# ethereum/pos-evolution

Measured on AMD Instinct MI355X. Metric: attestations aggregated/sec + get_head() p50 latency at 1M validators, higher is better.
Workload: dtype int32

## Files before the change

pos_evolution_amd/csrc/att_bodies.inc:

```
#include <algorithm>
#include "att_rules.h"
#include "kernels.h"
#include "wave64.h"

namespace posevo {

namespace {

constexpr uint32_t VAL_EQUIVOCATING_BIT = 0x04u;
constexpr uint32_t ERR_INVALID_ARG = 1, ERR_CAPACITY = 10, ERR_NO_COMMITTEES = 11;

struct Row9 { uint4 q[9]; };
__device__ __forceinline__ void load_row(Row9& r, const uint4* __restrict__ rows, uint32_t i)
{
    const uint4* p = rows + (size_t)9 * i;
#pragma unroll
    for (int k = 0; k < 9; ++k) r.q[k] = p[k];
}
__device__ __forceinline__ unsigned long long u64_of(uint32_t lo, uint32_t hi) { return ((unsigned long long)hi << 32) | lo; }
__device__ __forceinline__ unsigned long long row_slot(const Row9& r) { return u64_of(r.q[0].x, r.q[0].y); }
__device__ __forceinline__ unsigned long long row_index(const Row9& r) { return u64_of(r.q[0].z, r.q[0].w); }
__device__ __forceinline__ unsigned long long row_source_epoch(const Row9& r) { return u64_of(r.q[3].x, r.q[3].y); }
__device__ __forceinline__ unsigned long long row_target_epoch(const Row9& r) { return u64_of(r.q[5].z, r.q[5].w); }

// ... 204 lines not shown
                if (stalled) break;
                const unsigned long long mi = __ballot(valid && have_incl);
                const int first = mi ? __builtin_ctzll(mi) : 64;
                const bool take = valid && (int)lane <= first;
                base.a += wave_sum(take ? x0 >> 1 : 0ull);
                base.w += wave_sum(take ? x1 >> 1 : 0ull);
                base.b += wave_sum(take ? x2 >> 1 : 0ull);
                if (mi) break;
                hi -= 64;
                if (hi < 0) break;
            }
            if (stalled && lane == 0) atomicMax(&a.sync->err, ERR_STALL);
            if (lane == 0) {
                granule_store(&rec[bid].incl[0], ((base.a + tot_a24) << 1) | 1ull);
                granule_store(&rec[bid].incl[1], ((base.w + tot.w) << 1) | 1ull);
                granule_store(&rec[bid].incl[2], ((base.b + tot.b) << 1) | 1ull);
            }
        }
        if (lane == 0) { s_base[0] = base.a; s_base[1] = base.w; s_base[2] = base.b; }
    }
    __syncthreads();

    uint32_t g = 0;
    if (is_rep) {
        const unsigned long long ex_a = wgb.a + inc.a - v.a;
        g = (uint32_t)(s_base[0] & 0xFFFFFFull) + (uint32_t)(ex_a & 0xFFFFull);
        const uint32_t list_start = (uint32_t)((s_base[0] >> 24) + (ex_a >> 16));
        const uint32_t out_word = (uint32_t)(s_base[1] + wgb.w + inc.w - v.w);
        const uint32_t out_byte = (uint32_t)(s_base[2] + wgb.b + inc.b - v.b);
        AttGroup G;
        G.rep = i;
        G.n_atts = natts;
        G.list_start = list_start;
        G.cursor = 0;
        G.n_bits = nbits;
        G.out_word = out_word;
        G.out_byte = out_byte;
        G.table = st == ST_NO_TABLE ? NONE32 : table;
        G.pos = pos;
        G.size = size;
        G.member_base = mbase;
        G.sig_valid = FLAG_SIG_VALID;
        G.status_agg = (uint32_t)st;
        G.index_over = index_over;
        G.pad[0] = G.pad[1] = 0;
        a.grp[g] = G;
        UnionGroup u;
        u.list_start = list_start;
        u.n_atts = natts;
        u.n_bits = nbits;
        u.out_word = out_word;
        a.ug[g] = u;
        a.gid_of_row[i] = g;
        if (ok) atomicAdd(&a.crow_cnt[table][pos], 1u);
    }
    {
        const int32_t st_pk = att_committee_state_status(st, index_over != 0);
        const uint32_t e = (is_rep && st_pk != ST_OK && a.want_pk) ? (st_pk == ST_NO_TABLE ? ERR_NO_COMMITTEES : ERR_INVALID_ARG) : 0u;
        const uint32_t w_err = wave_max(e);
        const uint32_t w_size = wave_max(ok ? size : 0u);
        const uint32_t w_mis = wave_max((is_rep && bytes != 4 * words) ? ~g : 0u);
        const uint32_t w_r0 = (uint32_t)__builtin_popcountll(__ballot(ok && table == 0));
        const uint32_t w_r1 = (uint32_t)__builtin_popcountll(__ballot(ok && table == 1));
        const unsigned long long w_mem = wave_sum(ok ? (unsigned long long)size : 0ull);
        if (lane == 0) {
            PlanSync* S = a.sync;
            if (w_err) atomicMax(&S->err, w_err);
            if (w_size) atomicMax(&S->max_size, w_size);
            if (w_mis) atomicMax(&S->mis_key, w_mis);
            if (w_r0) atomicAdd(&S->rows_t[0], w_r0);
            if (w_r1) atomicAdd(&S->rows_t[1], w_r1);
            if (w_mem) atomicAdd(&S->total_members, w_mem);
        }
    }

    asm volatile("s_waitcnt vmcnt(0)" ::: "memory");
    __syncthreads();
    if (tid == 0) s_ticket = __hip_atomic_fetch_add(&a.sync->ticket, 1u, __ATOMIC_RELAXED, __HIP_MEMORY_SCOPE_AGENT);
    __syncthreads();
    if (s_ticket != nb - 1) return;

    PlanSync* S = a.sync;
    const uint32_t rows_t0 = word_load(&S->rows_t[0]), rows_t1 = word_load(&S->rows_t[1]);
    if (tid == 0) {
        const unsigned long long la = granule_load(&rec[nb - 1].incl[0]) >> 1, lw = granule_load(&rec[nb - 1].incl[1]) >> 1,
                                 lb = granule_load(&rec[nb - 1].incl[2]) >> 1;
        const uint32_t ng = (uint32_t)(la & 0xFFFFFFull);
        const uint32_t max_size = word_load(&S->max_size), mis_key = word_load(&S->mis_key);
        const unsigned long long total_members = granule_load(&S->total_members);
        uint32_t err = max(a.plan->error, word_load(&S->err));
        if (!err && (lb > a.out_arena_cap || lw > 0xFFFFFFFFull)) err = ERR_CAPACITY;
        uint32_t k = a.min_k, L = 0;
        {
            const unsigned long long k0 = max((unsigned long long)a.min_k, (total_members + a.target_slots - 1) / a.target_slots);
            uint32_t tasks = (uint32_t)((max_size + k0 - 1) / k0);
            if (tasks > (uint32_t)G1_WG) tasks = G1_WG;
            while ((1u << L) < tasks) ++L;
            while (L > 0 && ((unsigned long long)ng << L) > a.slot_cap) --L;
            k = max(a.min_k, (max_size + (1u << L) - 1) >> L);
            if (k == 0) k = 1;
        }
        AttPlan p;
        p.n_groups = err ? 0u : ng;
        p.n_slots = p.n_groups << L;
        p.k = k;
        p.log2_block = L;
        p.out_words = (uint32_t)lw;
        p.out_bytes = (uint32_t)min(lb, 0xFFFFFFFFull);
        p.error = err;
        p.packed_same = (mis_key != 0 && (~mis_key) + 1 < ng) ? 0u : 1u;
        p.n_rows_table[0] = rows_t0;
        p.n_rows_table[1] = rows_t1;
        p.n_rows_in = n;
        p.last_error = err;
        p.total_members = total_members;
        *a.plan = p;
        *a.plan_host = p;
    }
    for (int t = 0; t < 2; ++t) {
        if (!a.tables.t[t].valid || (t ? rows_t1 : rows_t0) == 0) continue;
        const uint32_t nc = a.tables.t[t].n_committees;
        const uint32_t per = (nc + 1 + PLAN_WG - 1) / PLAN_WG;
        const uint32_t b0 = min(tid * per, nc + 1), b1 = min(b0 + per, nc + 1);
        uint32_t sum = 0;
        for (uint32_t c = b0; c < b1; ++c) sum += c < nc ? word_load(&a.crow_cnt[t][c]) : 0u;
        const uint32_t incl = wave_incl_scan(sum);
        __syncthreads();
        if (lane == 63) s_scan[wave] = incl;
        __syncthreads();
        uint32_t run = incl - sum;
        for (uint32_t w = 0; w < wave; ++w) run += s_scan[w];
        for (uint32_t c = b0; c < b1; ++c) {
            const uint32_t cnt = c < nc ? word_load(&a.crow_cnt[t][c]) : 0u;
            a.crow_start[t][c] = run;
            a.crow_cursor[t][c] = run;
            if (c < nc && cnt) __hip_atomic_store(&a.crow_cnt[t][c], 0u, __ATOMIC_RELAXED, __HIP_MEMORY_SCOPE_AGENT);
            run += cnt;
        }
    }
    __syncthreads();
    for (uint32_t j = tid; j < nb; j += PLAN_WG)
#pragma unroll
        for (int q = 0; q < 3; ++q) { granule_store(&rec[j].agg[q], 0ull); granule_store(&rec[j].incl[q], 0ull); }
    if (tid == 0) {
        unsigned long long* z = reinterpret_cast<unsigned long long*>(S);
#pragma unroll
        for (int q = 0; q < (int)(sizeof(PlanSync) / 8); ++q) granule_store(z + q, 0ull);
    }
}
inline unsigned att_plan_blocks(const AttPlanArgs& a) { return std::max(1u, (a.n + PLAN_WG - 1) / PLAN_WG); }
}

namespace {
__device__ __forceinline__ void att_members_body(const uint32_t i , const MembersArgs& a)
{
    const uint4* __restrict__ rows = static_cast<const uint4*>(a.rows);
    uint32_t* __restrict__ tab = a.tab;
    uint32_t* __restrict__ cnt_tab = a.cnt_tab;
    const uint32_t* __restrict__ slot_of = a.slot_of;
    const uint32_t* __restrict__ rep_of = a.rep_of;
    const uint32_t* __restrict__ gid_of_row = a.gid_of_row;
    AttGroup* __restrict__ grp = a.grp;
    AttPlan* __restrict__ plan = a.plan;
    uint32_t* __restrict__ ubytes = a.ubytes;
    uint32_t* __restrict__ member_row = a.member_row;
    uint32_t* __restrict__ host_group_of = a.host_group_of;
    uint4* __restrict__ host_out_rows = static_cast<uint4*>(a.host_out_rows);
    uint32_t n = a.n;
    if (a.n_dev) n = min(n, *a.n_dev);
    if (i == 0 && n == 0) plan->error = 0;
    if (i >= n) return;
    const uint32_t slot = slot_of[i];
    if (plan->n_groups) {
        const uint32_t rep = rep_of[i];
        const uint32_t g = gid_of_row[rep];
        const uint4 q8 = rows[(size_t)9 * i + 8];
        if (host_group_of) host_group_of[i] = g;
        AttGroup& G = grp[g];
        const uint32_t p = G.list_start + atomicAdd(&G.cursor, 1u);
        ubytes[p] = q8.x;
        member_row[p] = i;
        if (!(q8.z & FLAG_SIG_VALID)) atomicAnd(&G.sig_valid, 0u);
        if (rep == i) {
            const uint32_t k = plan->k, L = plan->log2_block;
            const bool ok = G.status_agg == (uint32_t)ST_OK;
            G1Group d;
            d.member_start = G.member_base;
            d.n_members = ok ? G.size : 0u;
            d.bits_word = G.out_word;
            d.slot_base = g << L;
            d.n_tasks = ok ? (G.size + k - 1) / k : 0u;
            d.k = k | (G.table == 1 ? 0x80000000u : 0u);
            d.log2_block = L;
            d.out_base = g;
            a.g1[g] = d;
            if (ok) a.crow_list[G.table][atomicAdd(&a.crow_cursor[G.table][G.pos], 1u)] = g;
            if (host_out_rows) {
                uint4* o = host_out_rows + (size_t)9 * g;
#pragma unroll
                for (int k8 = 0; k8 < 8; ++k8) o[k8] = rows[(size_t)9 * i + k8];
                o[8] = make_uint4(G.out_byte, q8.y, q8.z, 0u);
            }
        }
    }
    tab[slot] = ATT_EMPTY;
    cnt_tab[slot] = 0;
    if (i == 0) plan->error = 0;
}
}

namespace {
__device__ __forceinline__ uint32_t find_block_dev(const BlockTableDev& bt, const uint4& r0, const uint4& r1)
{
    uint32_t h = r0.x & bt.root_mask;
    for (;;) {
        const uint32_t idx = bt.root_tab[h];
        if (idx == NONE32) return NONE32;
        const uint4* q = reinterpret_cast<const uint4*>(bt.roots + 32ull * idx);
        if (same4(q[0], r0) && same4(q[1], r1)) return idx;
        h = (h + 1) & bt.root_mask;
    }
}
struct Root2 { uint4 lo, hi; };
struct BlockStoreDev {
    const BlockTableDev& bt;
    __device__ __forceinline__ uint32_t find(const Root2& r) const { return find_block_dev(bt, r.lo, r.hi); }
    __device__ __forceinline__ uint32_t handle(uint32_t idx) const { return bt.pos_of_idx[idx]; }
    __device__ __forceinline__ unsigned long long slot_of(uint32_t idx) const { return bt.slot_pos[bt.pos_of_idx[idx]]; }
    __device__ __forceinline__ uint32_t ancestor(uint32_t idx, unsigned long long slot) const
    {
        uint32_t p = bt.pos_of_idx[idx];
        while (bt.slot_pos[p] > slot && bt.parent_pos[p] != NONE32) p = bt.parent_pos[p];
        return p;
    }
};
}

namespace {
__device__ __forceinline__ void att_validate_fc_body(const uint32_t g , const ValidateFcArgs& a)
{
    const uint4* __restrict__ rows = static_cast<const uint4*>(a.rows);
    const AttGroup* __restrict__ grp = a.grp;
    const AttPlan* __restrict__ plan = a.plan;
    const uint32_t cap = a.cap;
    const BlockTableDev& bt = a.bt;
    const FcCtx& fc = a.fc;
    const uint32_t* __restrict__ union_info = a.union_info;
    AttRow* __restrict__ out_rows = a.out_rows;
    int32_t* __restrict__ status_dev = a.status_dev;
    int32_t* __restrict__ status_host = a.status_host;
    uint32_t* __restrict__ count_host = a.count_host;
    uint32_t* __restrict__ err_host = a.err_host;
    const uint32_t ng = plan->n_groups;
    if (ng > cap) {
        if (g < ng) status_dev[g] = -1;
        if (g == 0) *err_host = ERR_CAPACITY;
        return;
    }
    if (g >= ng) return;
    const AttGroup G = grp[g];
    Row9 r;
    load_row(r, rows, G.rep);
    const unsigned long long slot = row_slot(r), tep = row_target_epoch(r), spe = fc.slots_per_epoch;
    const FcVerdict v = att_fork_choice_status(BlockStoreDev{bt}, (r.q[8].z & FLAG_FROM_BLOCK) != 0, slot, tep, Root2{r.q[6], r.q[7]},
                                               Root2{r.q[1], r.q[2]}, fc.cur_slot, fc.cur_epoch, fc.prev_epoch, spe);
    int32_t st = v.status;
    if (st == ST_OK) st = (int32_t)G.status_agg;
    const uint32_t cnt = union_info[2 * g], overlap = union_info[2 * g + 1];
    if (st == ST_OK) st = att_indexed_status(G.sig_valid != 0, overlap != 0, cnt);
    out_rows[g] = att_row_fork_choice(G.member_base, G.size, G.out_word, v.block, tep, slot, g, g);
    status_dev[g] = st;
    status_host[g] = st;
    if (count_host) count_host[g] = st == ST_OK ? cnt : 0u;
}
}

namespace {
__device__ __forceinline__ void lmd_vm_tables_body(const unsigned long long v , const LmdVmArgs& a)
{
    const AttRow* __restrict__ rows = a.rows;
    const TablesDev& tables = a.tables;
    const uint32_t* __restrict__ cs0 = a.crow_start[0];
    const uint32_t* __restrict__ cs1 = a.crow_start[1];
    const uint32_t* __restrict__ cl0 = a.crow_list[0];
    const uint32_t* __restrict__ cl1 = a.crow_list[1];
    const AttPlan* __restrict__ plan = a.plan;
    const uint32_t* __restrict__ bit_arena = a.bit_arena;
    const uint8_t* __restrict__ flags = a.flags;
    unsigned long long* __restrict__ vote_key = reinterpret_cast<unsigned long long*>(a.vote_key);
    uint32_t* __restrict__ vote_block = a.vote_block;
    uint32_t* __restrict__ vote_slot = a.vote_slot;
    const uint32_t* __restrict__ gates = a.gates;
    if (v >= a.n_val) return;
    uint32_t best_e = 0, best_order = NONE32, new_block = NONE32, new_slot = 0;
    bool loaded = false;
    for (int t = 0; t < 2; ++t) {
        if (!tables.t[t].valid || plan->n_rows_table[t] == 0) continue;
        const uint32_t c = tables.t[t].inv_comm[v];
        if (c == NONE32) continue;
        const uint32_t* crow_start = t ? cs1 : cs0;
        const uint32_t* crow_list = t ? cl1 : cl0;
        const uint32_t kb = crow_start[c], ke = crow_start[c + 1];
        if (kb == ke) continue;
        if (!loaded) {
            if (flags[v] & VAL_EQUIVOCATING_BIT) return;
            best_e = (uint32_t)(vote_key[v] >> 32);
            loaded = true;
        }
        const uint32_t i = tables.t[t].inv_pos[v];
        for (uint32_t k = kb; k < ke; ++k) {
            const AttRow r = rows[crow_list[k]];
            if (i >= r.n_bits) continue;
            if (gates[r.gate] != 0) continue;
            if (!((bit_arena[r.bits_word + (i >> 5)] >> (i & 31)) & 1u)) continue;
            if (r.epoch_p1 > best_e || (r.epoch_p1 == best_e && new_block != NONE32 && r.order < best_order)) {
                best_e = r.epoch_p1;
                best_order = r.order;
                new_block = r.block_idx;
                new_slot = r.slot;
            }
        }
    }
    if (new_block != NONE32) {
        vote_key[v] = ((unsigned long long)best_e << 32) | 0xFFFFFFFFull;
        vote_block[v] = new_block;
        if (vote_slot) vote_slot[v] = new_slot;
    }
}
}

}
```

pos_evolution_amd/csrc/engine_resident.cpp:

```cpp
#include "engine_internal.h"


using namespace posevo;

namespace posevo {

namespace {

struct RrLayout {
    AttPlan* plan;
    uint32_t *slot_of, *rep_of, *gid_of_row, *ubytes, *member_row;
    PlanSync* sync;
    PlanRec* rec;
    AttGroup* grp;
    UnionGroup* ug;
    G1Group* g1;
    AttRow *rows_fc, *rows_st;
    int32_t *status_fc, *status_st;
    uint32_t* cmpl;
    uint32_t *crow_start[2], *crow_cursor[2], *crow_cnt[2], *crow_list[2];
    size_t bytes;
};

RrLayout rr_layout(uint8_t* base, uint32_t cap_n, uint32_t cap_c)
{
    RrLayout L;
    size_t off = 0;
    auto take = [&](size_t bytes) {
        uint8_t* p = base ? base + off : nullptr;
        off = (off + bytes + 255) & ~size_t(255);
        return p;
    };
    L.plan = reinterpret_cast<AttPlan*>(take(sizeof(AttPlan)));
    L.slot_of = reinterpret_cast<uint32_t*>(take(4ull * cap_n));
    L.rep_of = reinterpret_cast<uint32_t*>(take(4ull * cap_n));
    L.gid_of_row = reinterpret_cast<uint32_t*>(take(4ull * cap_n));
    L.sync = reinterpret_cast<PlanSync*>(take(sizeof(PlanSync)));
    L.rec = reinterpret_cast<PlanRec*>(take(sizeof(PlanRec) * ((size_t)cap_n / PLAN_WG + 1)));
    L.ubytes = reinterpret_cast<uint32_t*>(take(4ull * cap_n));
    L.member_row = reinterpret_cast<uint32_t*>(take(4ull * cap_n));
    L.grp = reinterpret_cast<AttGroup*>(take(sizeof(AttGroup) * (size_t)cap_n));
    L.ug = reinterpret_cast<UnionGroup*>(take(sizeof(UnionGroup) * (size_t)cap_n));
    L.g1 = reinterpret_cast<G1Group*>(take(sizeof(G1Group) * (size_t)cap_n));
    L.rows_fc = reinterpret_cast<AttRow*>(take(sizeof(AttRow) * (size_t)cap_n));
    L.rows_st = reinterpret_cast<AttRow*>(take(sizeof(AttRow) * (size_t)cap_n));
    L.status_fc = reinterpret_cast<int32_t*>(take(4ull * cap_n));
    L.status_st = reinterpret_cast<int32_t*>(take(4ull * cap_n));
    L.cmpl = reinterpret_cast<uint32_t*>(take(4ull * cap_n));
    for (int t = 0; t < 2; ++t) {
        L.crow_start[t] = reinterpret_cast<uint32_t*>(take(4ull * (cap_c + 1)));
        L.crow_cursor[t] = reinterpret_cast<uint32_t*>(take(4ull * (cap_c + 1)));
        L.crow_cnt[t] = reinterpret_cast<uint32_t*>(take(4ull * (cap_c + 1)));
        L.crow_list[t] = reinterpret_cast<uint32_t*>(take(4ull * cap_n));
    }
    L.bytes = off;
    return L;
}

struct RrSet {
    DevBuf &tab, &rr, &bits, &info;
    uint32_t &rows_cap, &comm_cap, &tab_size;
};
RrSet rr_set(pe_engine::PipeArena& a, int set)
{
    if (set == 0) return RrSet{a.d_rr_tab, a.d_rr, a.d_res_bits, a.d_res_info, a.rr_rows_cap, a.rr_comm_cap, a.rr_tab_size};
    return RrSet{a.x_rr_tab, a.x_rr, a.x_res_bits, a.x_res_info, a.x_rows_cap, a.x_comm_cap, a.x_tab_size};
}
RrLayout rr_of(pe_engine::PipeArena& a, int set = 0)
{
    const RrSet s = rr_set(a, set);
    return rr_layout(s.rr.as<uint8_t>(), s.rows_cap, s.comm_cap);
}

int rr_ensure(pe_engine* h, pe_engine::PipeArena& arena, int set, uint32_t n, uint32_t n_comm)
{
    {
        const RrSet rs = rr_set(arena, set);
        if (n <= rs.rows_cap && n_comm <= rs.comm_cap && rs.rr.p && rs.tab.p) return PE_OK;
    }
    PE_TRY(flush_pending(h));
    HIP_TRY(h, hipDeviceSynchronize());
    uint32_t cap_n = 1024, cap_c = 64;
    for (int i = 0; i < h->n_arenas; ++i) {
        const RrSet o = rr_set(h->arena[i], set);
        cap_n = std::max(cap_n, o.rows_cap);
        cap_c = std::max(cap_c, o.comm_cap);
    }
    while (cap_n < n) cap_n *= 2;
    while (cap_c < n_comm) cap_c *= 2;
    uint32_t tab = 2048;
    while (tab < 2 * cap_n) tab <<= 1;
    const RrLayout L = rr_layout(nullptr, cap_n, cap_c);
    for (int i = 0; i < h->n_arenas; ++i) {
        pe_engine::PipeArena& other = h->arena[i];
        if (set != 0 && &other != &arena) continue;
        const RrSet a = rr_set(other, set);
        if (cap_n <= a.rows_cap && cap_c <= a.comm_cap && a.rr.p && a.tab.p) continue;
        a.rr.release();
        a.tab.release();
        HIP_TRY(h, a.rr.ensure(L.bytes));
        HIP_TRY(h, a.tab.ensure(8ull * tab));
        HIP_TRY(h, hipMemsetAsync(a.tab.p, 0xFF, 4ull * tab, h->stream));
        HIP_TRY(h, hipMemsetAsync(a.tab.as<uint8_t>() + 4ull * tab, 0, 4ull * tab, h->stream));
        HIP_TRY(h, hipMemsetAsync(a.rr.p, 0, L.bytes, h->stream));
        a.rows_cap = cap_n;
        a.comm_cap = cap_c;
        a.tab_size = tab;
    }
    HIP_TRY(h, hipStreamSynchronize(h->stream));
    return PE_OK;
}

int candidate_tables(pe_engine* h, TablesDev* out, CommitteeTable* tabs[2])
{
    memset(out, 0, sizeof(*out));
    out->slots_per_epoch = h->cfg.slots_per_epoch;
    const uint64_t cur = epoch_at_slot(h, current_slot(h));
    const uint64_t prev = cur > 0 ? cur - 1 : cur;
    const uint64_t epochs[2] = {cur, prev};
    for (int k = 0; k < 2; ++k) {
        tabs[k] = nullptr;
        out->t[k].epoch = epochs[k];
        if (k == 1 && prev == cur) continue;
        CommitteeTable* t = find_table(h, epochs[k]);
        if (!t) continue;
        if (!t->is_partition || t->n_val_at_load != h->n_val || !t->d_inv_comm.p)
            return fail(h, PE_ERR_INVALID_ARG,
                        "rows in device memory: the committee tables of the current / previous epoch must partition the "
                        "registry they were loaded for (use host rows otherwise)");
        tabs[k] = t;
        out->t[k].members = t->d_members.as<uint32_t>();
        out->t[k].offsets = t->d_offsets.as<uint32_t>();
        out->t[k].inv_comm = t->d_inv_comm.as<uint32_t>();
        out->t[k].inv_pos = t->d_inv_pos.as<uint32_t>();
        out->t[k].n_committees = t->n_committees;
        out->t[k].valid = 1;
// ... 82 lines not shown
    OutBlock ob(h);
    const size_t off_plan = ob.alloc(sizeof(AttPlan));
    const size_t off_rows = ob.alloc(sizeof(pe_attestation) * (size_t)n);
    const size_t off_gof = ob.alloc(4ull * n);
    const size_t off_obits = ob.alloc(words_cap * 4);
    const size_t off_oinfo = ob.alloc(8ull * n);
    const size_t off_opk = out_aggpk96 ? ob.alloc(96ull * n) : 0;
    G1Complement cm;
    bool by_cmpl = false;
    if (out_aggpk96 && !dev_partials && set == 0 && h->tune.committee_sums && !h->dist_ready())
        for (int t = 0; t < 2; ++t) {
            if (tabs[t]) PE_TRY(committee_sums_build_wanted(h, tabs[t]));
            if (tabs[t] && tabs[t]->sums_valid && tabs[t]->d_sums.p && tabs[t]->ev_sums) {
                cm.sums[t] = tabs[t]->d_sums.as<uint32_t>();
                cm.ev[t] = tabs[t]->ev_sums;
                by_cmpl = true;
            }
        }
    const size_t off_ocm = by_cmpl ? ob.alloc(4ull * n) : 0;
    PE_TRY(ob.ensure());
    if (by_cmpl) {
        cm.cmpl = L.cmpl;
        cm.info = RS.info.as<uint32_t>();
    }
    if (want_pk) {
        PE_TRY(ensure_quiesced_arenas(h, &pe_engine::PipeArena::d_partials, std::max<size_t>(PE_G1_PARTIAL_BYTES, (size_t)PE_G1_PARTIAL_BYTES * n)));
        PE_TRY(ensure_quiesced_arenas(h, &pe_engine::PipeArena::d_lane_partials, (size_t)G1_LANE_PARTIAL_BYTES * slot_cap));
        PE_TRY(ensure_quiesced(h, h->d_partials, std::max<size_t>(PE_G1_PARTIAL_BYTES, (size_t)PE_G1_PARTIAL_BYTES * n)));
        PE_TRY(ensure_quiesced(h, h->d_lane_partials, (size_t)G1_LANE_PARTIAL_BYTES * slot_cap));
    }
    lap.mark("ragg.1_reserve");
    *out_n_groups = 0;
    AttPlan* plan_host = ob.host<AttPlan>(off_plan);
    memset(plan_host, 0, sizeof(AttPlan));
    plan_host->error = 0xFFFFFFFFu;
    const MemKind arena_kind = arena_len ? mem_kind(bits_arena) : MemKind::Pageable;
    hipStream_t ms = h->stream;
    const bool pair_ok = h->held.active && h->held.arena != h->cur && set == 0 && !n_dev && hold_eligible(h);
    if (h->held.active && !pair_ok) PE_TRY(held_issue(h));
    if (set == 0) {
        if (!h->deferred.empty()) PE_TRY(run_deferred(h));
        if (A.side_used) HIP_TRY(h, hipStreamWaitEvent(ms, h->ev_join, 0));
        if (sig_batch_holds(h, h->cur)) PE_TRY(sig_batch_flush(h));
        if (A.leg_used) HIP_TRY(h, hipStreamWaitEvent(ms, A.ev_leg, 0));
        PE_TRY(aux_join(h, ms));
    }
    h->res_valid = false;
    h->rr.valid = false;
    const size_t deferred_before = h->deferred.size();
    struct Unwind {
        pe_engine* h; size_t keep; bool armed = true;
        ~Unwind() { if (armed) { h->rr.valid = false; if (h->deferred.size() > keep) h->deferred.resize(keep); } }
    } unwind{h, deferred_before};
    bool ingest_copies = false;
    if (arena_kind == MemKind::Pageable) {
        memcpy(st.host<uint8_t>(off_arena), bits_arena, arena_len);
        memset(st.host<uint8_t>(off_arena) + arena_len, 0, pad_at + 32 - arena_len);
        HIP_TRY(h, st.upload());
    } else if (arena_len) {
        if (arena_kind == MemKind::Device && (reinterpret_cast<uintptr_t>(bits_arena) & 15) == 0 && n > 0) ingest_copies = true;
        else HIP_TRY(h, hipMemcpyAsync(st.dev<uint8_t>(off_arena), bits_arena, arena_len,
                                       arena_kind == MemKind::Device ? hipMemcpyDeviceToDevice : hipMemcpyHostToDevice, ms));
    }
    lap.mark("ragg.2_bits");
    uint32_t* cnt_tab = RS.tab.as<uint32_t>() + RS.tab_size;
    const IngestArgs ia{d_rows, n, RS.tab.as<uint32_t>(), cnt_tab, RS.tab_size - 1, L.slot_of, arena_len, L.plan,
                        st.dev<uint8_t>(off_arena) + pad_at, n_dev, ingest_copies ? bits_arena : nullptr,
                        ingest_copies ? st.dev<uint8_t>(off_arena) : nullptr};
    AttPlanArgs pa;
    pa.rows = d_rows;
    pa.n = n;
    pa.n_dev = n_dev;
    pa.tab = RS.tab.as<uint32_t>();
    pa.cnt_tab = cnt_tab;
    pa.slot_of = L.slot_of;
    pa.rep_of = L.rep_of;
    pa.gid_of_row = L.gid_of_row;
    pa.grp = L.grp;
    pa.ug = L.ug;
    for (int t = 0; t < 2; ++t) {
        pa.crow_start[t] = L.crow_start[t];
        pa.crow_cursor[t] = L.crow_cursor[t];
        pa.crow_cnt[t] = L.crow_cnt[t];
    }
    pa.sync = L.sync;
    pa.rec = L.rec;
    pa.plan = L.plan;
    pa.plan_host = plan_host;
    pa.out_arena_cap = out_arena_cap;
    pa.target_slots = target;
    pa.slot_cap = slot_cap;
    pa.min_k = G1_MIN_K;
    pa.want_pk = want_pk ? 1u : 0u;
    pa.tables = tables;
    const MembersArgs ma{d_rows, n, RS.tab.as<uint32_t>(), cnt_tab, L.slot_of, L.rep_of, L.gid_of_row, L.grp, L.plan, L.ubytes,
                         L.member_row, group_of ? ob.host<uint32_t>(off_gof) : nullptr, ob.host<uint8_t>(off_rows), n_dev,
                         L.g1, {L.crow_cursor[0], L.crow_cursor[1]}, {L.crow_list[0], L.crow_list[1]}};
    const UnionArgs ua{L.ug, n, L.ubytes, st.dev<uint8_t>(off_arena), RS.bits.as<uint32_t>(), RS.info.as<uint32_t>(),
                       ob.host<uint32_t>(off_obits), ob.host<uint32_t>(off_oinfo), L.plan,
                       by_cmpl ? L.cmpl : nullptr, by_cmpl ? ob.host<uint32_t>(off_ocm) : nullptr, L.grp,
                       {cm.sums[0] ? 1u : 0u, cm.sums[1] ? 1u : 0u}};
    PE_TRY(launch_rows_paired(h, ia, pa, ma, ua));
    HIP_TRY(h, hipGetLastError());
    lap.mark("ragg.3_group_union");
    if (want_pk) {
        const bool on_side = h->pipelining && h->side_stream && h->stream == h->own_stream;
        h->last_agg_on_side = on_side;
        pe_engine::PipeArena* arena = &A;
        const uint32_t* d_points = h->d_points.as<uint32_t>();
        const uint32_t* d_union = RS.bits.as<uint32_t>();
        uint8_t* out_pk = out_aggpk96 ? ob.host<uint8_t>(off_opk) : nullptr;
        G1Plan bound;
        bound.n_groups = n;
        bound.n_slots = slot_cap;
        bound.n_partials = n;
        const G1Group* d_groups = L.g1;
        const AttPlan* d_plan = L.plan;
        uint32_t* dev_jac = dev_partials ? dev_partials : set == 0 ? h->keep_pk : nullptr;
        auto launch_g1 = [h, arena, d_points, tables, d_union, d_groups, bound, out_pk, on_side, d_plan, dev_jac, cm, by_cmpl]() -> int {
            hipStream_t gs = on_side ? h->side_stream : h->stream;
            if (on_side) {
                HIP_TRY(h, hipEventRecord(h->ev_fork, h->stream));
                HIP_TRY(h, hipStreamWaitEvent(gs, h->ev_fork, 0));
            }
            if (on_side) {
                if (arena->side_used) HIP_TRY(h, hipStreamWaitEvent(gs, h->ev_join, 0));
            } else {
                g1_stream_guard(h, gs);
            }
            PE_TRY(launch_g1_planned(h, d_points, tables.t[0].members, d_union, d_groups, bound, out_pk, dev_jac, gs,
                                     on_side ? h->fin_stream : gs, on_side ? &arena->d_partials : nullptr,
                                     on_side ? &arena->d_lane_partials : nullptr, d_plan, tables.t[1].members, 0,
                                     by_cmpl ? &cm : nullptr));
            if (on_side) {
                HIP_TRY(h, hipEventRecord(h->ev_join, h->g1_tail()));
                h->side_busy = true;
                h->side_ever = true;
                arena->side_used = true;
            }
            return PE_OK;
        };
        if (on_side && h->streaming && !g1_chain_idle(h)) h->deferred.push_back(launch_g1);
        else PE_TRY(launch_g1());
        lap.mark("ragg.4_g1");
    }
    for (int t = 0; t < 2; ++t)
        if (tabs[t]) tabs[t]->stamp = ++h->table_stamp;
    unwind.armed = false;
    h->rr.valid = true;
    h->rr.arena = h->cur;
    h->rr.set = set;
    h->rr.n_in = n;
    h->rr.rows = d_rows;
    h->rr.tables = tables;
    ++h->rr.generation;
    h->rr.n_groups = NONE32;
    const size_t base = ob.base;
    const int ai = h->cur;
    const uint64_t gen = h->rr.generation;
    auto complete = [h, ai, base, off_plan, off_rows, off_gof, off_obits, off_oinfo, off_opk, off_ocm, by_cmpl, n, out_atts,
                     out_n_groups, group_of, out_bits_arena, out_aggpk96, out_count, gen]() -> int {
        const uint8_t* pin = h->arena[ai].h_pin.as<uint8_t>() + base;
        const AttPlan P = *reinterpret_cast<const AttPlan*>(pin + off_plan);
        if (P.error) return plan_error_to_status(h, P.error == 0xFFFFFFFFu ? 1u : P.error, "pe_aggregate (rows in device memory)");
        const uint32_t ng = P.n_groups;
        if (ng > n) return fail(h, PE_ERR_NO_DEVICE, "k_att_plan returned more groups than rows");
// ... 18 lines not shown
        h->last_cmpl_groups = 0;
        if (by_cmpl) {
            const uint32_t* ocm = reinterpret_cast<const uint32_t*>(pin + off_ocm);
            for (uint32_t g = 0; g < ng; ++g) h->last_cmpl_groups += ocm[g] != NONE32 ? 1u : 0u;
        }
        return PE_OK;
    };
    HostLap lap2(&h->trace);
    const int rc = finish_call(h, st, ob, complete);
    lap2.mark("ragg.5_wait_outputs");
    return rc;
}

int resident_plan_dev(pe_engine* h, const AttPlan** out)
{
    if (!h->rr.valid) return fail(h, PE_ERR_STATE, "no aggregate over rows in device memory on this handle");
    *out = rr_of(h->arena[h->rr.arena], h->rr.set).plan;
    return PE_OK;
}

int resident_parts(pe_engine* h, ResidentParts* out)
{
    if (!h->rr.valid) return fail(h, PE_ERR_STATE, "no aggregate over rows in device memory on this handle");
    pe_engine::PipeArena& RA = h->arena[h->rr.arena];
    const RrLayout L = rr_of(RA, h->rr.set);
    const RrSet RS = rr_set(RA, h->rr.set);
    out->rows = h->rr.rows;
    out->grp = L.grp;
    out->plan = L.plan;
    out->res_bits = RS.bits.as<uint32_t>();
    out->res_info = RS.info.as<uint32_t>();
    out->n_in = h->rr.n_in;
    return PE_OK;
}

int resident_lists(pe_engine* h, const UnionGroup** ug, const uint32_t** member_row)
{
    if (!h->rr.valid) return fail(h, PE_ERR_STATE, "no aggregate over rows in device memory on this handle");
    const RrLayout L = rr_of(h->arena[h->rr.arena], h->rr.set);
    *ug = L.ug;
    *member_row = L.member_row;
    return PE_OK;
}

int resident_precheck(pe_engine* h, const char* who)
{
    if (!h->rr.valid) return fail(h, PE_ERR_STATE, std::string(who) + ": PE_ROWS_RESIDENT without a pe_aggregate over rows in device memory on this handle");
    TablesDev now;
    CommitteeTable* tabs[2];
    PE_TRY(candidate_tables(h, &now, tabs));
    for (int t = 0; t < 2; ++t)
        if (now.t[t].epoch != h->rr.tables.t[t].epoch || now.t[t].valid != h->rr.tables.t[t].valid ||
            now.t[t].members != h->rr.tables.t[t].members)
            return fail(h, PE_ERR_STATE, std::string(who) + ": the store's clock or its committee tables changed since the resident pe_aggregate: aggregate again");
    return PE_OK;
}

int on_attestation_resident(pe_engine* h, uint32_t cap, int32_t* status, uint32_t* out_count)
{
    PE_TRY(resident_precheck(h, "pe_on_attestation_batch"));
    if (cap == 0) return PE_OK;
    if (h->held.active && (h->held.arena != h->cur || h->held.have_fc || h->held.have_head)) PE_TRY(held_issue(h));
    HostLap lap(&h->trace);
    PE_TRY(refresh_tree(h));
    pe_engine::PipeArena& RA = h->arena[h->rr.arena];
    const RrLayout L = rr_of(RA, h->rr.set);
    const RrSet RS = rr_set(RA, h->rr.set);
    Stage st(h);
    OutBlock ob(h);
    const size_t off_status = ob.alloc(4ull * cap);
    const size_t off_count = ob.alloc(4ull * cap);
    const size_t off_err = ob.alloc(16);
    PE_TRY(ob.ensure());
    *ob.host<uint32_t>(off_err) = 0;
    FcCtx fc;
    fc.cur_slot = current_slot(h);
    fc.cur_epoch = epoch_at_slot(h, fc.cur_slot);
    fc.prev_epoch = fc.cur_epoch > 0 ? fc.cur_epoch - 1 : 0;
    fc.slots_per_epoch = h->cfg.slots_per_epoch;
    const uint32_t n_launch = std::max<uint32_t>(h->rr.n_in, 1);
    memset(ob.host<int32_t>(off_status), 0, 4ull * cap);
    memset(ob.host<uint32_t>(off_count), 0, 4ull * cap);
    const ValidateFcArgs va{h->rr.rows, L.grp, L.plan, n_launch, cap, block_table_dev(h), fc, RS.info.as<uint32_t>(), L.rows_fc,
                            L.status_fc, ob.host<int32_t>(off_status), ob.host<uint32_t>(off_count), ob.host<uint32_t>(off_err)};
    const LmdVmArgs la{L.rows_fc, h->rr.tables, {L.crow_start[0], L.crow_start[1]}, {L.crow_list[0], L.crow_list[1]}, L.plan,
                       RS.bits.as<uint32_t>(), h->d_flags.as<uint8_t>(), h->n_val, h->d_vote_key.as<uint64_t>(),
                       h->d_vote_block.as<uint32_t>(), h->cfg.vote_expiry_slots ? h->d_vote_slot.as<uint32_t>() : nullptr,
                       reinterpret_cast<const uint32_t*>(L.status_fc)};
    if (hold_eligible(h) && h->rr.arena == h->cur && h->rr.set == 0 && h->n_val) {
        h->held.validate = va;
        h->held.lmd = la;
        h->held.have_fc = true;
        h->held.active = true;
        h->held.arena = h->cur;
    } else {
        if (h->held.active) PE_TRY(held_issue(h));
        {
            ProfScope ps(h, PE_KERNEL_ATT_VALIDATE);
            launch_att_validate_fc(h->stream, va);
        }
        ProfScope ps(h, PE_KERNEL_LMD);
        launch_lmd_vm_tables(h->stream, la);
    }
    HIP_TRY(h, hipGetLastError());
    lap.mark("ratt.1_launch");
    const size_t base = ob.base;
    const int ai = h->cur;
    auto complete = [h, ai, base, off_status, off_count, off_err, cap, status, out_count]() -> int {
        const uint8_t* pin = h->arena[ai].h_pin.as<uint8_t>() + base;
        const uint32_t err = *reinterpret_cast<const uint32_t*>(pin + off_err);
        if (err) return plan_error_to_status(h, err, "pe_on_attestation_batch (PE_ROWS_RESIDENT)");
        memcpy(status, pin + off_status, 4ull * cap);
        if (out_count) memcpy(out_count, pin + off_count, 4ull * cap);
        return PE_OK;
    };
    HostLap lap2(&h->trace);
    const int rc = finish_call(h, st, ob, complete);
    lap2.mark("ratt.2_wait_outputs");
    return rc;
}

int process_attestation_resident(pe_engine* h, const pe_state_ctx* sc, uint32_t cap, int32_t* status, uint64_t* out_numerators)
{
    PE_TRY(resident_precheck(h, "pe_process_attestation_batch"));
    if (cap == 0) return PE_OK;
    const uint64_t spe = h->cfg.slots_per_epoch;
    if (spe > 64) return fail(h, PE_ERR_CAPACITY, "PE_ROWS_RESIDENT: SLOTS_PER_EPOCH above 64");
    uint32_t tip;
    if (!find_block(h, to_root(sc->chain_tip_root), &tip)) return fail(h, PE_ERR_UNKNOWN_ROOT, "chain tip unknown");
    HostLap lap(&h->trace);
    PE_TRY(refresh_tree(h));
    pe_engine::PipeArena& RA = h->arena[h->rr.arena];
    const RrLayout L = rr_of(RA, h->rr.set);
    const RrSet RS = rr_set(RA, h->rr.set);
    Stage st(h);
    StateCtxDev S;
    memset(&S, 0, sizeof(S));
    S.slot = sc->slot;
    S.cur_epoch = sc->slot / spe;
    S.prev_epoch = S.cur_epoch > 0 ? S.cur_epoch - 1 : 0;
    S.slots_per_epoch = spe;
    S.min_inclusion_delay = h->cfg.min_attestation_inclusion_delay;
    S.sqrt_spe = isqrt64(spe);
    S.cj_epoch = sc->current_justified_epoch;
    S.pj_epoch = sc->previous_justified_epoch;
    memcpy(S.cj_root, sc->current_justified_root, 32);
    memcpy(S.pj_root, sc->previous_justified_root, 32);
    S.base_reward_per_increment = sc->base_reward_per_increment;
    {
        uint32_t cur = tip;
        for (uint64_t j = spe; j-- > 0;) {
            if (S.slot + j < spe) { S.head_blk[j] = NONE32; continue; }
            cur = get_ancestor(h, cur, S.slot + j - spe);
            S.head_blk[j] = cur;
        }
        S.tgt_blk[0] = get_ancestor(h, tip, S.cur_epoch * spe);
        S.tgt_blk[1] = get_ancestor(h, tip, S.prev_epoch * spe);
    }
    OutBlock ob(h);
    const size_t off_err = ob.alloc(16);
    const size_t off_status = ob.alloc(4ull * cap);
    const size_t off_num = ob.alloc(8ull * cap);
    PE_TRY(ob.ensure());
    *ob.host<uint32_t>(off_err) = 0;
    memset(ob.host<int32_t>(off_status), 0, 4ull * cap);
    memset(ob.host<uint64_t>(off_num), 0, 8ull * cap);
    const uint32_t n_launch = std::max<uint32_t>(h->rr.n_in, 1);
    hipStream_t ss = state_stream_begin(h, true, n_launch);
    {
        ProfScope ps(h, PE_KERNEL_ATT_VALIDATE, ss);
        launch_att_validate_state(ss, h->rr.rows, L.grp, L.plan, n_launch, cap, block_table_dev(h), S,
// ... 30 lines not shown
```

pos_evolution_amd/csrc/kernels.h:

```cpp
#pragma once
#include <hip/hip_runtime.h>
#include <stdint.h>

namespace posevo {

template <int TAG>
static bool first_use_on_this_device()
{
    static bool done[64] = {false};
    int dev = 0;
    (void)hipGetDevice(&dev);
    if (dev < 0 || dev >= 64) return true;
    if (done[dev]) return false;
    done[dev] = true;
    return true;
}

constexpr uint32_t NONE32 = 0xFFFFFFFFu;
constexpr int G1_ROW_WORDS = 32;
constexpr int G2_WG_SLOTS = 128;
constexpr int G1_WG = 256;
constexpr int G1_LANE_PARTIAL_BYTES = 208;
constexpr int TREE_MAX_BLOCKS = 8192;
constexpr int VOTES_MAX_WG = 256;
// ... 81 lines not shown
                                uint32_t* vote_block, uint32_t* vote_slot = nullptr, const uint32_t* gates = nullptr);
void launch_participation(hipStream_t s, const AttRow* rows, uint32_t n_rows, const uint32_t* members,
                          const uint32_t* bit_arena, const uint16_t* eff_increments,
                          uint64_t base_reward_per_increment, uint32_t* part_cur_words,
                          uint32_t* part_prev_words, uint64_t* numerators, const uint32_t* numerator_slot,
                          const uint32_t* gates = nullptr);
struct UnionGroup {
    uint32_t list_start;
    uint32_t n_atts;
    uint32_t n_bits;
    uint32_t out_word;
};

constexpr uint32_t ATT_EMPTY = 0xFFFFFFFFu;
struct TableDev {
    uint64_t epoch;
    const uint32_t* members;
    const uint32_t* offsets;
    const uint32_t* inv_comm;
    const uint32_t* inv_pos;
    uint32_t n_committees;
    uint32_t valid;
};
struct TablesDev {
    TableDev t[2];
    uint64_t slots_per_epoch;
};
struct AttPlan {
    uint32_t n_groups;
    uint32_t n_slots;
    uint32_t k, log2_block;
    uint32_t out_words, out_bytes;
    uint32_t error;
    uint32_t packed_same;
    uint32_t n_rows_table[2];
    uint32_t n_rows_in;
    uint32_t last_error;
    unsigned long long total_members;
};
struct AttGroup {
    uint32_t rep;
    uint32_t n_atts, list_start, cursor;
    uint32_t n_bits, out_word, out_byte;
    uint32_t table;
    uint32_t pos, size, member_base;
    uint32_t sig_valid;
    uint32_t status_agg;
    uint32_t index_over;
    uint32_t pad[2];
};
struct BlockTableDev {
    const uint32_t* root_tab;
    uint32_t root_mask;
    const uint8_t* roots;
    const unsigned long long* slot_pos;
    const uint32_t* parent_pos;
    const uint32_t* pos_of_idx;
    uint32_t n_blocks;
};
struct FcCtx {
    unsigned long long cur_slot, cur_epoch, prev_epoch, slots_per_epoch;
};
struct StateCtxDev {
    unsigned long long slot, cur_epoch, prev_epoch, slots_per_epoch, min_inclusion_delay, sqrt_spe;
    unsigned long long cj_epoch, pj_epoch;
    uint8_t cj_root[32], pj_root[32];
    uint32_t tgt_blk[2];
    uint32_t head_blk[64];
    unsigned long long base_reward_per_increment;
};
struct PlanSync {
    uint32_t ticket;
    uint32_t max_size;
    uint32_t rows_t[2];
    uint32_t mis_key;
    uint32_t err;
    uint32_t pad[2];
    unsigned long long total_members, pad2[3];
};
struct PlanRec {
    unsigned long long agg[3], incl[3], pad[2];
};
constexpr uint32_t PLAN_WG = 256;
constexpr uint32_t PLAN_MAX_ROWS = 1u << 24;
struct AttPlanArgs {
    const void* rows; uint32_t n; const uint32_t* n_dev;
    const uint32_t* tab; const uint32_t* cnt_tab; const uint32_t* slot_of;
    uint32_t* rep_of; uint32_t* gid_of_row;
    AttGroup* grp; UnionGroup* ug;
    uint32_t* crow_start[2]; uint32_t* crow_cursor[2]; uint32_t* crow_cnt[2];
    PlanSync* sync; PlanRec* rec;
    AttPlan* plan; AttPlan* plan_host;
    uint64_t out_arena_cap; uint32_t target_slots, slot_cap, min_k, want_pk;
    TablesDev tables;
};
void launch_att_plan(hipStream_t s, const AttPlanArgs& a);
void launch_att_pack(hipStream_t s, const void* rows, const AttGroup* grp, const AttPlan* plan, const uint32_t* res_bits,
                     const uint32_t* res_info, uint32_t slots, uint32_t wps, uint32_t* send);
void launch_att_unpack(hipStream_t s, const uint32_t* recv, uint32_t world, uint32_t slots, uint32_t wps, void* out_rows,
                       uint32_t* out_bits, uint32_t* n_dev, uint32_t* err_host);
void launch_att_validate_state(hipStream_t s, const void* rows, const AttGroup* grp, const AttPlan* plan, uint32_t n_bound,
                               uint32_t cap, BlockTableDev bt, const StateCtxDev& st, const uint32_t* union_info,
                               AttRow* out_rows, int32_t* status_dev, int32_t* status_host, uint32_t* err_host);
void launch_participation_tables(hipStream_t s, const AttRow* rows, TablesDev tables, uint32_t* const crow_start[2],
                                 uint32_t* const crow_list[2], const AttPlan* plan, const uint32_t* bit_arena,
                                 const uint16_t* eff_increments, uint64_t base_reward_per_increment,
                                 uint32_t* part_cur_words, uint32_t* part_prev_words, uint64_t* numerators,
                                 const uint32_t* gates, uint32_t cap);

struct IngestArgs {
    const void* rows; uint32_t n;
    uint32_t* tab; uint32_t* cnt_tab;
    uint32_t tab_mask;
    uint32_t* slot_of;
    uint64_t arena_len; AttPlan* plan;
    void* arena_pad32;
    const uint32_t* n_dev;
    const void* arena_src; void* arena_dst;
};
struct ValidateFcArgs {
    const void* rows; const AttGroup* grp; const AttPlan* plan;
    uint32_t n_bound, cap;
    BlockTableDev bt; FcCtx fc;
    const uint32_t* union_info; AttRow* out_rows; int32_t* status_dev; int32_t* status_host; uint32_t* count_host;
    uint32_t* err_host;
};
struct LmdVmArgs {
    const AttRow* rows; TablesDev tables; const uint32_t* crow_start[2]; const uint32_t* crow_list[2];
    const AttPlan* plan; const uint32_t* bit_arena; const uint8_t* flags; uint64_t n_val; uint64_t* vote_key;
    uint32_t* vote_block; uint32_t* vote_slot; const uint32_t* gates;
};
struct MembersArgs {
    const void* rows; uint32_t n; uint32_t* tab; uint32_t* cnt_tab; const uint32_t* slot_of; const uint32_t* rep_of;
    const uint32_t* gid_of_row; AttGroup* grp; AttPlan* plan; uint32_t* ubytes; uint32_t* member_row;
    uint32_t* host_group_of; void* host_out_rows; const uint32_t* n_dev;
    G1Group* g1; uint32_t* crow_cursor[2]; uint32_t* crow_list[2];
};
struct VotesArgs {
    const uint32_t* vote_block; const uint64_t* eff_balance; const uint8_t* flags; uint64_t n_val;
    uint32_t filter_slashed; const uint32_t* pos_of_idx; uint32_t n_blocks; uint64_t* direct; VoteTotals* totals;
    const uint32_t* vote_slot; uint32_t min_vote_slot;
};
struct UnionArgs {
    const UnionGroup* groups; uint32_t n_groups; const uint32_t* att_bytes;
    const uint8_t* bit_arena;
    uint32_t* out_arena;
    uint32_t* out_info;
    uint32_t* host_arena; uint32_t* host_info;
    const AttPlan* plan_dev;
    uint32_t* cmpl; uint32_t* host_cmpl; const AttGroup* grp; uint32_t sums_ok[2];
};
struct TreeArgs {
    TreeDev tree; uint64_t* direct; const VoteTotals* totals; uint64_t ov_balance, ov_num; int use_override;
    uint32_t justified_pos, boost_pos; uint64_t slots_per_epoch, boost_percent, balance_increment;
    uint64_t* weights_by_idx; uint32_t* head_idx; int clear_direct;
};
struct RemapArgs {
    uint32_t* vote_block; uint64_t n_val;
    const uint32_t* map; uint32_t n_old;
    unsigned long long* counts;
};
constexpr uint32_t VOTE_PRUNED = 0xFFFFFFFEu;
constexpr int REMAP_WG = 256;
constexpr unsigned REMAP_MAX_WG = 256;
void launch_votes_remap(hipStream_t s, const RemapArgs& a);
void launch_att_ingest(hipStream_t s, const IngestArgs& a);
void launch_att_validate_fc(hipStream_t s, const ValidateFcArgs& a);
void launch_lmd_vm_tables(hipStream_t s, const LmdVmArgs& a);
void launch_att_members(hipStream_t s, const MembersArgs& a);
void launch_votes(hipStream_t s, const VotesArgs& a, int lean);
void votes_clear_exchange(hipStream_t s, uint64_t* direct, uint32_t n_blocks, VoteTotals* totals);
void launch_bits_union(hipStream_t s, const UnionArgs& a);
void launch_tree(hipStream_t s, const TreeArgs& a, int lean);
bool launch_pair_ingest_validate(hipStream_t s, const IngestArgs& rows_next, const ValidateFcArgs& fc_prev);
bool launch_pair_plan_lmd(hipStream_t s, const AttPlanArgs& rows_next, const LmdVmArgs& fc_prev);
bool launch_pair_members_votes(hipStream_t s, const MembersArgs& rows_next, const VotesArgs& fc_prev);
bool launch_pair_union_tree(hipStream_t s, const UnionArgs& rows_next, const TreeArgs& fc_prev);
void pair_kernels_preload();

struct SlashRow {
    uint32_t bits_byte;
    uint32_t n_bits;
    uint32_t source, target;
    uint32_t id;
    uint32_t pad[3];
};
struct SlashTable {
    const uint32_t* inv_comm;
    const uint32_t* inv_pos;
    const uint32_t* crow_start;
};
struct SlashArgs {
    const SlashRow* rows;
    const SlashTable* tables; uint32_t n_tables;
    const uint32_t* crow_list;
    const uint8_t* bits;
    unsigned long long* rec; uint32_t* ids; uint32_t history; uint64_t n_val;
    uint32_t* counter;
    uint32_t* evidence; uint32_t cap;
    uint8_t* flags;
};
constexpr int SLASH_NV = 4;
void launch_slash_scan(hipStream_t s, const SlashArgs& a);

struct SlashRowsArgs {
    const void* rows;
    const AttGroup* grp; uint32_t n_groups;
    uint64_t window; uint32_t history;
    uint32_t max_data, tab_mask;
    uint32_t slot_of_table[2];
    uint8_t* data; uint32_t* count; uint32_t* tab;
    int32_t* status;
    uint32_t* err;
// ... 212 lines not shown
```

Measured before the change: 7.038 billion.

## Add per-committee single-row fast path records for LMD vote scan

The plan kernel tags each committee as having zero, one, or many attestation rows, and now scans committee counts in chunks of sixteen with a carried block prefix instead of a variable per-thread span. The validate kernel writes a compact 32-byte record for committees that have exactly one row. The LMD vote kernel then reads that record with two 16-byte loads instead of indirecting through crow_start, crow_list and the full row array. The zeroing of the per-block records is also moved earlier and spread across threads. This adds extra memory for tags and records and extra stores during validation.

```diff
diff --git a/pos_evolution_amd/csrc/att_bodies.inc b/pos_evolution_amd/csrc/att_bodies.inc
--- a/pos_evolution_amd/csrc/att_bodies.inc
+++ b/pos_evolution_amd/csrc/att_bodies.inc
@@ -310,6 +310,9 @@
 
     PlanSync* S = a.sync;
     const uint32_t rows_t0 = word_load(&S->rows_t[0]), rows_t1 = word_load(&S->rows_t[1]);
+    for (uint32_t j = tid; j + 1 < nb; j += PLAN_WG)
+#pragma unroll
+        for (int q = 0; q < 3; ++q) { granule_store(&rec[j].agg[q], 0ull); granule_store(&rec[j].incl[q], 0ull); }
     if (tid == 0) {
         const unsigned long long la = granule_load(&rec[nb - 1].incl[0]) >> 1, lw = granule_load(&rec[nb - 1].incl[1]) >> 1,
                                  lb = granule_load(&rec[nb - 1].incl[2]) >> 1;
@@ -348,29 +351,53 @@
     for (int t = 0; t < 2; ++t) {
         if (!a.tables.t[t].valid || (t ? rows_t1 : rows_t0) == 0) continue;
         const uint32_t nc = a.tables.t[t].n_committees;
-        const uint32_t per = (nc + 1 + PLAN_WG - 1) / PLAN_WG;
-        const uint32_t b0 = min(tid * per, nc + 1), b1 = min(b0 + per, nc + 1);
-        uint32_t sum = 0;
-        for (uint32_t c = b0; c < b1; ++c) sum += c < nc ? word_load(&a.crow_cnt[t][c]) : 0u;
-        const uint32_t incl = wave_incl_scan(sum);
-        __syncthreads();
-        if (lane == 63) s_scan[wave] = incl;
-        __syncthreads();
-        uint32_t run = incl - sum;
-        for (uint32_t w = 0; w < wave; ++w) run += s_scan[w];
-        for (uint32_t c = b0; c < b1; ++c) {
-            const uint32_t cnt = c < nc ? word_load(&a.crow_cnt[t][c]) : 0u;
-            a.crow_start[t][c] = run;
-            a.crow_cursor[t][c] = run;
-            if (c < nc && cnt) __hip_atomic_store(&a.crow_cnt[t][c], 0u, __ATOMIC_RELAXED, __HIP_MEMORY_SCOPE_AGENT);
-            run += cnt;
+        uint32_t* __restrict__ cnt_t = a.crow_cnt[t];
+        uint32_t* __restrict__ start_t = a.crow_start[t];
+        uint32_t* __restrict__ cursor_t = a.crow_cursor[t];
+        uint32_t* __restrict__ tag_t = a.crow_tag[t];
+        uint32_t carry = 0;
+        for (uint32_t base = 0; base <= nc; base += PLAN_WG * CROW_SCAN_PER) {
+            const uint32_t c0 = base + tid * CROW_SCAN_PER;
+            uint32_t cnt[CROW_SCAN_PER];
+#pragma unroll
+            for (int j = 0; j < CROW_SCAN_PER; ++j) cnt[j] = word_load(&cnt_t[min(c0 + j, nc - 1)]);
+            uint32_t sum = 0;
+#pragma unroll
+            for (int j = 0; j < CROW_SCAN_PER; ++j) {
+                if (c0 + j >= nc) cnt[j] = 0;
+                sum += cnt[j];
+            }
+            const uint32_t incl = wave_incl_scan(sum);
+            __syncthreads();
+            if (lane == 63) s_scan[wave] = incl;
+            __syncthreads();
+            uint32_t run = carry + incl - sum, all = 0;
+#pragma unroll
+            for (uint32_t w = 0; w < (uint32_t)PLAN_WAVES; ++w) {
+                const uint32_t x = s_scan[w];
+                if (w < wave) run += x;
+                all += x;
+            }
+            carry += all;
+#pragma unroll
+            for (int j = 0; j < CROW_SCAN_PER; ++j) {
+                const uint32_t c = c0 + j;
+                if (c <= nc) {
+                    start_t[c] = run;
+                    cursor_t[c] = run;
+                    if (c < nc) {
+                        tag_t[c] = cnt[j] == 0 ? NONE32 : cnt[j] == 1 ? CROW_ONE : CROW_MULTI;
+                        if (cnt[j]) __hip_atomic_store(&cnt_t[c], 0u, __ATOMIC_RELAXED, __HIP_MEMORY_SCOPE_AGENT);
+                    }
+                }
+                run += cnt[j];
+            }
         }
     }
     __syncthreads();
-    for (uint32_t j = tid; j < nb; j += PLAN_WG)
-#pragma unroll
-        for (int q = 0; q < 3; ++q) { granule_store(&rec[j].agg[q], 0ull); granule_store(&rec[j].incl[q], 0ull); }
     if (tid == 0) {
+#pragma unroll
+        for (int q = 0; q < 3; ++q) { granule_store(&rec[nb - 1].agg[q], 0ull); granule_store(&rec[nb - 1].incl[q], 0ull); }
         unsigned long long* z = reinterpret_cast<unsigned long long*>(S);
 #pragma unroll
         for (int q = 0; q < (int)(sizeof(PlanSync) / 8); ++q) granule_store(z + q, 0ull);
@@ -465,6 +492,14 @@
 }
 
 namespace {
+__device__ __forceinline__ void crow_rec_store(const ValidateFcArgs& a, const AttGroup& G, const AttRow& row, const bool live)
+{
+    if (G.status_agg != (uint32_t)ST_OK || G.table > 1u) return;
+    if (a.crow_tag[G.table][G.pos] != CROW_ONE) return;
+    uint4* p = reinterpret_cast<uint4*>(a.crow_rec[G.table] + G.pos);
+    p[0] = make_uint4(row.bits_word, row.n_bits, row.block_idx, row.epoch_p1);
+    p[1] = make_uint4(row.order, row.slot, live ? 1u : 0u, 0u);
+}
 __device__ __forceinline__ void att_validate_fc_body(const uint32_t g , const ValidateFcArgs& a)
 {
     const uint4* __restrict__ rows = static_cast<const uint4*>(a.rows);
@@ -481,7 +516,10 @@
     uint32_t* __restrict__ err_host = a.err_host;
     const uint32_t ng = plan->n_groups;
     if (ng > cap) {
-        if (g < ng) status_dev[g] = -1;
+        if (g < ng) {
+            status_dev[g] = -1;
+            crow_rec_store(a, grp[g], AttRow{}, false);
+        }
         if (g == 0) *err_host = ERR_CAPACITY;
         return;
     }
@@ -496,7 +534,9 @@
     if (st == ST_OK) st = (int32_t)G.status_agg;
     const uint32_t cnt = union_info[2 * g], overlap = union_info[2 * g + 1];
     if (st == ST_OK) st = att_indexed_status(G.sig_valid != 0, overlap != 0, cnt);
-    out_rows[g] = att_row_fork_choice(G.member_base, G.size, G.out_word, v.block, tep, slot, g, g);
+    const AttRow row = att_row_fork_choice(G.member_base, G.size, G.out_word, v.block, tep, slot, g, g);
+    out_rows[g] = row;
+    crow_rec_store(a, G, row, st == ST_OK);
     status_dev[g] = st;
     status_host[g] = st;
     if (count_host) count_host[g] = st == ST_OK ? cnt : 0u;
@@ -512,6 +552,10 @@
     const uint32_t* __restrict__ cs1 = a.crow_start[1];
     const uint32_t* __restrict__ cl0 = a.crow_list[0];
     const uint32_t* __restrict__ cl1 = a.crow_list[1];
+    const uint32_t* __restrict__ ct0 = a.crow_tag[0];
+    const uint32_t* __restrict__ ct1 = a.crow_tag[1];
+    const CrowRec* __restrict__ cr0 = a.crow_rec[0];
+    const CrowRec* __restrict__ cr1 = a.crow_rec[1];
     const AttPlan* __restrict__ plan = a.plan;
     const uint32_t* __restrict__ bit_arena = a.bit_arena;
     const uint8_t* __restrict__ flags = a.flags;
@@ -520,22 +564,37 @@
     uint32_t* __restrict__ vote_slot = a.vote_slot;
     const uint32_t* __restrict__ gates = a.gates;
     if (v >= a.n_val) return;
+    if (plan->n_groups == 0) return;
     uint32_t best_e = 0, best_order = NONE32, new_block = NONE32, new_slot = 0;
     bool loaded = false;
     for (int t = 0; t < 2; ++t) {
         if (!tables.t[t].valid || plan->n_rows_table[t] == 0) continue;
         const uint32_t c = tables.t[t].inv_comm[v];
         if (c == NONE32) continue;
-        const uint32_t* crow_start = t ? cs1 : cs0;
-        const uint32_t* crow_list = t ? cl1 : cl0;
-        const uint32_t kb = crow_start[c], ke = crow_start[c + 1];
-        if (kb == ke) continue;
+        const uint32_t tag = (t ? ct1 : ct0)[c];
+        const uint4* rp = reinterpret_cast<const uint4*>((t ? cr1 : cr0) + c);
+        const uint4 ra = rp[0], rb = rp[1];
+        if (tag == NONE32) continue;
         if (!loaded) {
             if (flags[v] & VAL_EQUIVOCATING_BIT) return;
             best_e = (uint32_t)(vote_key[v] >> 32);
             loaded = true;
         }
         const uint32_t i = tables.t[t].inv_pos[v];
+        if (tag == CROW_ONE) {
+            if (i >= ra.y || rb.z == 0) continue;
+            if (!((bit_arena[ra.x + (i >> 5)] >> (i & 31)) & 1u)) continue;
+            if (ra.w > best_e || (ra.w == best_e && new_block != NONE32 && rb.x < best_order)) {
+                best_e = ra.w;
+                best_order = rb.x;
+                new_block = ra.z;
+                new_slot = rb.y;
+            }
+            continue;
+        }
+        const uint32_t* crow_start = t ? cs1 : cs0;
+        const uint32_t* crow_list = t ? cl1 : cl0;
+        const uint32_t kb = crow_start[c], ke = crow_start[c + 1];
         for (uint32_t k = kb; k < ke; ++k) {
             const AttRow r = rows[crow_list[k]];
             if (i >= r.n_bits) continue;
diff --git a/pos_evolution_amd/csrc/engine_resident.cpp b/pos_evolution_amd/csrc/engine_resident.cpp
--- a/pos_evolution_amd/csrc/engine_resident.cpp
+++ b/pos_evolution_amd/csrc/engine_resident.cpp
@@ -19,6 +19,8 @@
     int32_t *status_fc, *status_st;
     uint32_t* cmpl;
     uint32_t *crow_start[2], *crow_cursor[2], *crow_cnt[2], *crow_list[2];
+    uint32_t* crow_tag[2];
+    CrowRec* crow_rec[2];
     size_t bytes;
 };
 
@@ -52,6 +54,8 @@
         L.crow_cursor[t] = reinterpret_cast<uint32_t*>(take(4ull * (cap_c + 1)));
         L.crow_cnt[t] = reinterpret_cast<uint32_t*>(take(4ull * (cap_c + 1)));
         L.crow_list[t] = reinterpret_cast<uint32_t*>(take(4ull * cap_n));
+        L.crow_tag[t] = reinterpret_cast<uint32_t*>(take(4ull * (cap_c + 1)));
+        L.crow_rec[t] = reinterpret_cast<CrowRec*>(take(sizeof(CrowRec) * ((size_t)cap_c + 1)));
     }
     L.bytes = off;
     return L;
@@ -300,6 +304,7 @@
         pa.crow_start[t] = L.crow_start[t];
         pa.crow_cursor[t] = L.crow_cursor[t];
         pa.crow_cnt[t] = L.crow_cnt[t];
+        pa.crow_tag[t] = L.crow_tag[t];
     }
     pa.sync = L.sync;
     pa.rec = L.rec;
@@ -484,11 +489,13 @@
     memset(ob.host<int32_t>(off_status), 0, 4ull * cap);
     memset(ob.host<uint32_t>(off_count), 0, 4ull * cap);
     const ValidateFcArgs va{h->rr.rows, L.grp, L.plan, n_launch, cap, block_table_dev(h), fc, RS.info.as<uint32_t>(), L.rows_fc,
-                            L.status_fc, ob.host<int32_t>(off_status), ob.host<uint32_t>(off_count), ob.host<uint32_t>(off_err)};
+                            L.status_fc, ob.host<int32_t>(off_status), ob.host<uint32_t>(off_count), ob.host<uint32_t>(off_err),
+                            {L.crow_tag[0], L.crow_tag[1]}, {L.crow_rec[0], L.crow_rec[1]}};
     const LmdVmArgs la{L.rows_fc, h->rr.tables, {L.crow_start[0], L.crow_start[1]}, {L.crow_list[0], L.crow_list[1]}, L.plan,
                        RS.bits.as<uint32_t>(), h->d_flags.as<uint8_t>(), h->n_val, h->d_vote_key.as<uint64_t>(),
                        h->d_vote_block.as<uint32_t>(), h->cfg.vote_expiry_slots ? h->d_vote_slot.as<uint32_t>() : nullptr,
-                       reinterpret_cast<const uint32_t*>(L.status_fc)};
+                       reinterpret_cast<const uint32_t*>(L.status_fc), {L.crow_tag[0], L.crow_tag[1]},
+                       {L.crow_rec[0], L.crow_rec[1]}};
     if (hold_eligible(h) && h->rr.arena == h->cur && h->rr.set == 0 && h->n_val) {
         h->held.validate = va;
         h->held.lmd = la;
diff --git a/pos_evolution_amd/csrc/kernels.h b/pos_evolution_amd/csrc/kernels.h
--- a/pos_evolution_amd/csrc/kernels.h
+++ b/pos_evolution_amd/csrc/kernels.h
@@ -187,13 +187,17 @@
     unsigned long long agg[3], incl[3], pad[2];
 };
 constexpr uint32_t PLAN_WG = 256;
+constexpr uint32_t CROW_ONE = 1u, CROW_MULTI = 0xFFFFFFFEu;
+struct alignas(32) CrowRec { uint32_t bits_word, n_bits, block_idx, epoch_p1, order, slot, live, pad; };
+static_assert(sizeof(CrowRec) == 32, "two 16-byte loads");
+constexpr int CROW_SCAN_PER = 16;
 constexpr uint32_t PLAN_MAX_ROWS = 1u << 24;
 struct AttPlanArgs {
     const void* rows; uint32_t n; const uint32_t* n_dev;
     const uint32_t* tab; const uint32_t* cnt_tab; const uint32_t* slot_of;
     uint32_t* rep_of; uint32_t* gid_of_row;
     AttGroup* grp; UnionGroup* ug;
-    uint32_t* crow_start[2]; uint32_t* crow_cursor[2]; uint32_t* crow_cnt[2];
+    uint32_t* crow_start[2]; uint32_t* crow_cursor[2]; uint32_t* crow_cnt[2]; uint32_t* crow_tag[2];
     PlanSync* sync; PlanRec* rec;
     AttPlan* plan; AttPlan* plan_host;
     uint64_t out_arena_cap; uint32_t target_slots, slot_cap, min_k, want_pk;
@@ -229,11 +233,13 @@
     BlockTableDev bt; FcCtx fc;
     const uint32_t* union_info; AttRow* out_rows; int32_t* status_dev; int32_t* status_host; uint32_t* count_host;
     uint32_t* err_host;
+    const uint32_t* crow_tag[2]; CrowRec* crow_rec[2];
 };
 struct LmdVmArgs {
     const AttRow* rows; TablesDev tables; const uint32_t* crow_start[2]; const uint32_t* crow_list[2];
     const AttPlan* plan; const uint32_t* bit_arena; const uint8_t* flags; uint64_t n_val; uint64_t* vote_key;
     uint32_t* vote_block; uint32_t* vote_slot; const uint32_t* gates;
+    const uint32_t* crow_tag[2]; const CrowRec* crow_rec[2];
 };
 struct MembersArgs {
     const void* rows; uint32_t n; uint32_t* tab; uint32_t* cnt_tab; const uint32_t* slot_of; const uint32_t* rep_of;
```

After: 6.584 billion. -6.4%, worse.
